# flavie-yuan-liu/DL_attack_on_ImageNet

Measured on AMD Instinct MI355X. Metric: adversarial images/sec (ADiL learning step, classifier included), higher is better.
Workload: dtype bf16; 1 GPU; ADiL learn_dictionary_a step vs resnet50, 512 images/GPU, 50 atoms, 224x224, bf16 image streams + fp32 D/V master, loss=logits, clean pseudo-labels computed once per image and cached (1 fwd + 1 bwd per step; result-neutral, profiles/r03_label_stability.md); global_batch=512, atoms=50, inner_iters=131, parallelism=dp1: images+codes sharded, D replicated, 1 all-reduce(grad_d)/step

## Files before the change

### dl_attack_on_imagenet_amd/_lib.py

```python
import ctypes
import os
from ctypes import c_float, c_int, c_size_t, c_void_p

_PKG = os.path.dirname(os.path.abspath(__file__))
LIBPATH = os.environ.get("ADIL_HIP_LIBRARY") or os.path.join(_PKG, "lib", "libadil_hip.so")

SIGNATURES = {
    "adil_abi_version": (c_int, []),
    "adil_max_atoms": (c_int, []),
    "adil_grad_workspace_bytes": (c_size_t, [c_int, c_int, c_int]),
    "adil_grad_code_rows": (c_int, [c_int]),
    "adil_grad_slab_offset": (c_size_t, [c_int, c_int, c_int]),
    "adil_pack_codes": (c_int, [c_void_p, c_void_p, c_int, c_int, c_void_p, c_void_p, c_void_p, c_int, c_void_p, c_int, c_int,
                                c_void_p]),
    "adil_gather_images": (c_int, [c_void_p, c_int, c_void_p, c_void_p, c_int, c_int, c_int, c_void_p]),
    "adil_spd_inverse": (c_int, [c_void_p, c_int, c_void_p, c_void_p]),
    "adil_synth": (c_int, [c_void_p, c_void_p, c_void_p, c_void_p, c_int, c_int, c_int, c_int, c_float, c_int, c_void_p]),
    "adil_images_to_u8": (c_int, [c_void_p, c_int, c_void_p, c_size_t, c_void_p, c_void_p]),
    "adil_synth_store": (c_int, [c_void_p, c_void_p, c_void_p, c_void_p, c_void_p, c_int, c_int, c_int, c_int, c_float, c_int,
                                 c_void_p]),
    "adil_synth_fp8": (c_int, [c_void_p, c_void_p, c_void_p, c_void_p, c_int, c_int, c_int, c_int, c_float, c_float, c_int,
                               c_void_p]),
    "adil_dict_to_fp8": (c_int, [c_void_p, c_size_t, c_void_p, c_void_p]),
    "adil_adamw_clamp_fp8": (c_int, [c_void_p, c_void_p, c_int, c_void_p, c_void_p, c_size_t, c_float, c_float, c_float,
                                     c_float, c_float, c_float, c_float, c_float, c_void_p, c_void_p, c_void_p, c_void_p]),
    "adil_synth_fp8_packed": (c_int, [c_void_p, c_void_p, c_void_p, c_void_p, c_int, c_int, c_int, c_int, c_float, c_float,
                                      c_int, c_void_p]),
    "adil_grad": (c_int, [c_void_p, c_void_p, c_void_p, c_void_p, c_void_p, c_void_p, c_int, c_int, c_int, c_int, c_int,
                          c_void_p, c_size_t, c_void_p, c_void_p]),
    "adil_adamw_clamp": (c_int, [c_void_p, c_void_p, c_int, c_void_p, c_void_p, c_size_t, c_float, c_float, c_float,
                                 c_float, c_float, c_float, c_float, c_float, c_void_p, c_void_p, c_void_p]),
    "adil_zstep": (c_int, [c_void_p, c_void_p, c_void_p, c_void_p, c_void_p, c_int, c_int, c_int, c_float, c_float,
                           c_float, c_float, c_float, c_float, c_float, c_float, c_void_p, c_void_p, c_float, c_void_p,
                           c_void_p, c_void_p]),
    "adil_zstep_codes_slab_bytes": (c_size_t, [c_int, c_int, c_int]),
    "adil_zstep_codes": (c_int, [c_void_p, c_void_p, c_void_p, c_void_p, c_void_p, c_int, c_int, c_int, c_float, c_float,
                                 c_float, c_float, c_float, c_float, c_float, c_float, c_void_p, c_void_p, c_float, c_void_p,
                                 c_void_p, c_void_p, c_size_t, c_void_p, c_void_p]),
    "adil_adamw_l1ball": (c_int, [c_void_p, c_void_p, c_void_p, c_int, c_void_p, c_void_p, c_int, c_int, c_float, c_float,
                                  c_float, c_float, c_float, c_float, c_float, c_void_p, c_void_p, c_float, c_void_p, c_void_p,
                                  c_void_p, c_int, c_int, c_void_p]),
    "adil_atom_l1ball_project": (c_int, [c_void_p, c_int, c_int, c_int, c_float, c_void_p]),
    "adil_l1ball_project": (c_int, [c_void_p, c_int, c_int, c_float, c_void_p]),
    "adil_l2ball_project": (c_int, [c_void_p, c_int, c_int, c_float, c_void_p]),
    "adil_ista_step": (c_int, [c_void_p, c_void_p, c_size_t, c_float, c_float, c_void_p]),
    "adil_atom_workspace_bytes": (c_size_t, [c_int, c_int]),
    "adil_atom_norms": (c_int, [c_void_p, c_int, c_int, c_void_p, c_void_p, c_size_t, c_void_p]),
    "adil_atom_scale": (c_int, [c_void_p, c_int, c_int, c_void_p, c_int, c_void_p]),
    "adil_gram_workspace_bytes": (c_size_t, [c_int, c_int]),
    "adil_gram": (c_int, [c_void_p, c_int, c_int, c_void_p, c_void_p, c_size_t, c_void_p]),
    "adil_dict_rightmul": (c_int, [c_void_p, c_void_p, c_int, c_int, c_void_p, c_void_p]),
    "adil_image_metrics": (c_int, [c_void_p, c_void_p, c_int, c_int, c_int, c_void_p, c_void_p, c_void_p]),
    "adil_affine_act_fwd": (c_int, [c_void_p, c_void_p, c_void_p, c_void_p, c_void_p, c_size_t, c_int, c_int, c_int, c_int,
                                    c_void_p]),
    "adil_affine_act_bwd": (c_int, [c_void_p, c_void_p, c_void_p, c_void_p, c_void_p, c_size_t, c_int, c_int, c_int, c_int,
                                    c_void_p]),
    "adil_stem_conv_fwd": (c_int, [c_void_p, c_int, c_void_p, c_float, c_float, c_float, c_float, c_float, c_float,
                                   c_void_p, c_void_p, c_void_p, c_int, c_int, c_int, c_void_p]),
    "adil_maxpool_fwd": (c_int, [c_void_p, c_void_p, c_void_p, c_int, c_int, c_int, c_int, c_void_p]),
    "adil_stem_pool_bwd": (c_int, [c_void_p, c_void_p, c_void_p, c_void_p, c_void_p, c_int, c_int, c_int, c_int, c_void_p]),
    "adil_pw_conv_fwd": (c_int, [c_void_p, c_void_p, c_void_p, c_void_p, c_void_p, c_void_p, c_int, c_int, c_int, c_int,
                                 c_void_p, c_void_p, c_int, c_int, c_void_p]),
    "adil_pw_conv_bwd": (c_int, [c_void_p, c_void_p, c_void_p, c_void_p, c_void_p, c_void_p, c_void_p, c_int, c_int, c_int,
                                 c_int, c_void_p, c_void_p, c_void_p, c_void_p, c_int, c_int, c_void_p]),
    "adil_pw_conv_bwd_tile": (c_int, [c_void_p, c_void_p, c_void_p, c_void_p, c_void_p, c_void_p, c_void_p, c_int, c_int, c_int,
                                      c_int, c_void_p, c_void_p, c_void_p, c_void_p, c_int, c_int, c_void_p, c_int]),
    "adil_pw_route_policy": (c_int, [c_int]),
    "adil_pw_join_fwd": (c_int, [c_void_p, c_void_p, c_void_p, c_void_p, c_void_p, c_void_p, c_void_p, c_void_p, c_void_p,
                                 c_void_p, c_void_p, c_void_p, c_int, c_int, c_int, c_void_p]),
    "adil_pw_join_bwd": (c_int, [c_void_p, c_void_p, c_void_p, c_void_p, c_void_p, c_void_p, c_void_p, c_void_p, c_void_p,
                                 c_void_p, c_void_p, c_void_p, c_void_p, c_int, c_int, c_int, c_void_p]),
    "adil_conv3x3": (c_int, [c_void_p, c_void_p, c_void_p, c_int, c_int, c_int, c_int, c_int, c_void_p]),
    "adil_conv3x3_loop": (c_int, [c_int]),
    "adil_conv3x3_s2_fwd": (c_int, [c_void_p, c_void_p, c_void_p, c_int, c_int, c_int, c_int, c_int, c_void_p]),
    "adil_conv3x3_s2_bwd": (c_int, [c_void_p, c_void_p, c_void_p, c_int, c_int, c_int, c_int, c_int, c_void_p]),
    "adil_dw3x3_fwd": (c_int, [c_void_p, c_void_p, c_void_p, c_void_p, c_int, c_int, c_int, c_int, c_int, c_int, c_void_p]),
    "adil_dw3x3_bwd": (c_int, [c_void_p, c_void_p, c_void_p, c_void_p, c_int, c_int, c_int, c_int, c_int, c_int, c_void_p]),
    "adil_pw8_fwd": (c_int, [c_void_p, c_void_p, c_void_p, c_void_p, c_void_p, c_void_p, c_int, c_int, c_int, c_int, c_void_p]),
    "adil_pw8_bwd": (c_int, [c_void_p, c_void_p, c_void_p, c_void_p, c_void_p, c_int, c_int, c_int, c_int, c_void_p]),
    "adil_stem_conv_bwd": (c_int, [c_void_p, c_void_p, c_float, c_float, c_float, c_void_p, c_int, c_int, c_int, c_int,
                                   c_void_p]),
    "adil_first3x3_fwd": (c_int, [c_void_p, c_int, c_void_p, c_float, c_float, c_float, c_float, c_float, c_float,
                                  c_void_p, c_void_p, c_void_p, c_int, c_int, c_int, c_int, c_void_p]),
    "adil_first3x3_bwd": (c_int, [c_void_p, c_void_p, c_void_p, c_void_p, c_float, c_float, c_float, c_void_p, c_int, c_int,
                                  c_int, c_int, c_int, c_void_p]),
    "adil_pool_head_fwd": (c_int, [c_void_p, c_void_p, c_void_p, c_void_p, c_void_p, c_int, c_int, c_int, c_int, c_void_p]),
    "adil_pool_head_bwd": (c_int, [c_void_p, c_void_p, c_void_p, c_void_p, c_int, c_int, c_int, c_int, c_void_p]),
    "adil_bn_pool_head_fwd": (c_int, [c_void_p] * 7 + [c_int, c_int, c_int, c_int, c_void_p]),
    "adil_bn_pool_head_bwd": (c_int, [c_void_p] * 7 + [c_int, c_int, c_int, c_int, c_void_p]),
    "adil_dense1x1_fwd": (c_int, [c_void_p, c_void_p, c_void_p, c_void_p, c_void_p, c_void_p, c_void_p, c_int, c_int, c_int,
                                  c_int, c_void_p]),
    "adil_dense1x1_bwd": (c_int, [c_void_p, c_void_p, c_void_p, c_void_p, c_void_p, c_void_p, c_void_p, c_void_p, c_int, c_int,
                                  c_int, c_int, c_void_p]),
    "adil_dense3x3_fwd": (c_int, [c_void_p, c_void_p, c_void_p, c_int, c_int, c_int, c_int, c_int, c_void_p]),
    "adil_dense3x3_bwd": (c_int, [c_void_p, c_void_p, c_void_p, c_int, c_int, c_int, c_int, c_int, c_void_p]),
    "adil_dense1x1_fwd_ld": (c_int, [c_void_p, c_int, c_void_p, c_void_p, c_void_p, c_void_p, c_void_p, c_void_p, c_int, c_int,
                                     c_int, c_int, c_int, c_void_p]),
    "adil_dense1x1_bwd_ld": (c_int, [c_void_p, c_int, c_void_p, c_int, c_void_p, c_void_p, c_void_p, c_int, c_void_p, c_void_p,
                                     c_void_p, c_int, c_int, c_int, c_int, c_int, c_int, c_void_p]),
    "adil_dense3x3_fwd_ld": (c_int, [c_void_p, c_int, c_void_p, c_void_p, c_int, c_int, c_int, c_int, c_int, c_int, c_void_p]),
    "adil_dense3x3_bwd_ld": (c_int, [c_void_p, c_int, c_void_p, c_void_p, c_int, c_int, c_int, c_int, c_int, c_int, c_void_p]),
    "adil_dense_transition_fwd": (c_int, [c_void_p, c_void_p, c_void_p, c_void_p, c_void_p, c_int, c_int, c_int, c_int, c_int,
                                          c_void_p]),
    "adil_dense_transition_bwd": (c_int, [c_void_p, c_int, c_void_p, c_void_p, c_void_p, c_void_p, c_void_p, c_int, c_int,
                                          c_int, c_int, c_int, c_void_p]),
}

ABI_VERSION = 8
_lib = None


class AdilLibraryError(RuntimeError):
    pass


def load(path: str = None) -> ctypes.CDLL:
    global _lib
    if _lib is not None and path is None:
        return _lib
    p = path or LIBPATH
    import torch
    if not os.path.exists(p):
        raise AdilLibraryError(
            f"HIP kernel library not found at {p}. Build it with `python -m dl_attack_on_imagenet_amd.build` "
            "(needs hipcc). There is no CPU fallback for the ADiL hot path.")
    try:
        lib = ctypes.CDLL(p)
    except OSError as e:
        raise AdilLibraryError(f"cannot load {p}: {e}") from e
    for name, (res, args) in SIGNATURES.items():
        try:
            fn = getattr(lib, name)
        except AttributeError as e:
            raise AdilLibraryError(f"{p} does not export `{name}` (stale build?)") from e
        fn.restype, fn.argtypes = res, args
    if lib.adil_abi_version() != ABI_VERSION:
        raise AdilLibraryError(f"ABI mismatch: library {lib.adil_abi_version()} != binding {ABI_VERSION}")
    if path is None:
        _lib = lib
    return lib


def check(rc: int, what: str) -> None:
    if rc != 0:
        names = {-1: "ADIL_EINVAL (bad argument)", -2: "ADIL_EWORKSPACE (workspace too small)"}
        raise AdilLibraryError(f"{what} failed: {names.get(rc, f'hipError_t {rc}')}")
```

### dl_attack_on_imagenet_amd/csrc/adil_stem.hip

```cpp
#include <hip/hip_runtime.h>
#include <stdint.h>

#include "adil_common.h"
#include "adil_hip.h"
#include "adil_mfma.h"

namespace {

struct StemNorm { float mean[3]; float inv_std[3]; };

#define ST_T 16
#define ST_ROWS (2 * ST_T + 5)
#define ST_COLS 40
#define ST_RS (ST_COLS * 4 + 8)
#define ST_K 224
#define ST_WS (ST_K + 8)
#define ST_OS 72

template <typename TX>
__global__ __launch_bounds__(256) __attribute__((amdgpu_waves_per_eu(3))) void stem_conv_fwd_kernel(const TX* __restrict__ x, const bf16_t* __restrict__ wf,
                                                            StemNorm nm, const float* __restrict__ scale,
                                                            const float* __restrict__ shift, bf16_t* __restrict__ y,
                                                            int H, int W, int OH, int OW) {
    __shared__ __attribute__((aligned(16))) bf16_t smem[ST_ROWS * ST_RS + 64 * ST_WS];
    static_assert(4 * 32 * ST_OS <= ST_ROWS * ST_RS + 64 * ST_WS, "output scratch must fit in the tile buffers");
    bf16_t* sin = smem;
    bf16_t* sw = smem + ST_ROWS * ST_RS;
    bf16_t* sout = smem;
    const int tid = threadIdx.x, lane = tid & 63, w = tid >> 6, c = lane & 31, h = lane >> 5;
    const int n = blockIdx.z, oh0 = blockIdx.y * ST_T, ow0 = blockIdx.x * ST_T;
    {
        u32x4 wv[7];
#pragma unroll
        for (int j = 0; j < 7; ++j) wv[j] = *reinterpret_cast<const u32x4*>(wf + (size_t)(tid + 256 * j) * 8);
#pragma unroll
        for (int j = 0; j < 7; ++j) {
            const int q = tid + 256 * j, co = q / 28, off = q - co * 28;
            *reinterpret_cast<u32x4*>(sw + co * ST_WS + off * 8) = wv[j];
        }
    }
    const TX* xn = x + (size_t)n * 3 * H * W;
    constexpr int NPOS = (ST_ROWS * ST_COLS + 255) / 256;
    float raw[NPOS][3], okm[NPOS];
#pragma unroll
    for (int j = 0; j < NPOS; ++j) {
        const int pos = tid + 256 * j < ST_ROWS * ST_COLS ? tid + 256 * j : ST_ROWS * ST_COLS - 1;
        const int row = pos / ST_COLS, col = pos - row * ST_COLS;
        const int ih = 2 * oh0 - 3 + row, iw = 2 * ow0 - 3 + col;
        const bool ok = (ih >= 0) && (ih < H) && (iw >= 0) && (iw < W);
        const size_t at = (size_t)(ok ? ih : 0) * W + (ok ? iw : 0);
        okm[j] = ok ? 1.0f : 0.0f;
        raw[j][0] = Elem<TX>::load(xn, at);
        raw[j][1] = Elem<TX>::load(xn + (size_t)H * W, at);
        raw[j][2] = Elem<TX>::load(xn + (size_t)2 * H * W, at);
    }
#pragma unroll
    for (int j = 0; j < NPOS; ++j) {
        const int pos = tid + 256 * j;
        const int row = pos / ST_COLS, col = pos - row * ST_COLS;
        const float v0 = (raw[j][0] - nm.mean[0]) * nm.inv_std[0] * okm[j];
        const float v1 = (raw[j][1] - nm.mean[1]) * nm.inv_std[1] * okm[j];
        const float v2 = (raw[j][2] - nm.mean[2]) * nm.inv_std[2] * okm[j];
        u32x2 t;
        t[0] = pack2_bf16(v0, v1);
        t[1] = pack2_bf16(v2, 0.0f);
        if (pos < ST_ROWS * ST_COLS) *reinterpret_cast<u32x2*>(sin + row * ST_RS + col * 4) = t;
    }
    lds_sync();
    f32x16 acc[2][2];
#pragma unroll
    for (int p = 0; p < 2; ++p)
#pragma unroll
        for (int ct = 0; ct < 2; ++ct)
#pragma unroll
            for (int r = 0; r < 16; ++r) acc[p][ct][r] = 0.0f;
    const int prow = c >> 4, pcol = c & 15;
#pragma unroll 1
    for (int kh = 0; kh < 7; ++kh) {
#pragma unroll
        for (int g = 0; g < 2; ++g) {
            bf16x8 a[2], b[2];
#pragma unroll
            for (int ct = 0; ct < 2; ++ct) a[ct] = lds8(sw + (ct * 32 + c) * ST_WS + kh * 32 + 16 * g + 8 * h);
#pragma unroll
            for (int p = 0; p < 2; ++p) {
                const int orow = 2 * (2 * w + p) + prow;
                b[p] = lds8(sin + (2 * orow + kh) * ST_RS + 8 * pcol + 16 * g + 8 * h);
            }
#pragma unroll
            for (int p = 0; p < 2; ++p)
#pragma unroll
                for (int ct = 0; ct < 2; ++ct) mma16(acc[p][ct], a[ct], b[p]);
        }
    }
    lds_sync();
    bf16_t* so = sout + w * 32 * ST_OS;
#pragma unroll
    for (int p = 0; p < 2; ++p) {
#pragma unroll
        for (int ct = 0; ct < 2; ++ct) {
#pragma unroll
            for (int q = 0; q < 4; ++q) {
                const int co = ct * 32 + 8 * q + 4 * h;
                float v[4];
#pragma unroll
                for (int j = 0; j < 4; ++j) v[j] = fmaxf(acc[p][ct][4 * q + j] * scale[co + j] + shift[co + j], 0.0f);
                u32x2 t;
                t[0] = pack2_bf16(v[0], v[1]);
                t[1] = pack2_bf16(v[2], v[3]);
                *reinterpret_cast<u32x2*>(so + c * ST_OS + co) = t;
            }
        }
#pragma unroll
        for (int i = 0; i < 4; ++i) {
            const int id = lane + 64 * i, px = id >> 3, ch = (id & 7) * 8;
            const int oh = oh0 + 2 * (2 * w + p) + (px >> 4), ow = ow0 + (px & 15);
            const u32x4 t = *reinterpret_cast<const u32x4*>(so + px * ST_OS + ch);
            if (oh < OH && ow < OW) *reinterpret_cast<u32x4*>(y + (((size_t)n * OH + oh) * OW + ow) * 64 + ch) = t;
        }
    }
}


__global__ __launch_bounds__(256) void maxpool_fwd_kernel(const bf16_t* __restrict__ y, bf16_t* __restrict__ p,
                                                          uint8_t* __restrict__ idx, int B, int OH, int OW, int PH, int PW,
                                                          int C8) {
    const size_t i = (size_t)blockIdx.x * 256 + threadIdx.x;
    const size_t total = (size_t)B * PH * PW * C8;
    if (i >= total) return;
    const int c8 = (int)(i % C8);
    size_t r = i / C8;
    const int pw = (int)(r % PW); r /= PW;
    const int ph = (int)(r % PH);
    const int n = (int)(r / PH);
    float best[8];
    unsigned bi[8];
#pragma unroll
    for (int j = 0; j < 8; ++j) { best[j] = -INFINITY; bi[j] = 0xffu; }
#pragma unroll
    for (int kh = 0; kh < 3; ++kh) {
        const int oh = 2 * ph - 1 + kh;
#pragma unroll
        for (int kw = 0; kw < 3; ++kw) {
            const int ow = 2 * pw - 1 + kw;
            if (oh >= 0 && oh < OH && ow >= 0 && ow < OW) {
                const u32x4 t = *reinterpret_cast<const u32x4*>(y + ((((size_t)n * OH + oh) * OW + ow) * C8 + c8) * 8);
                float f[8];
                unpack8(t, f);
#pragma unroll
                for (int j = 0; j < 8; ++j) {
                    const bool take = (f[j] > best[j]) || (f[j] != f[j]) || (bi[j] == 0xffu);
                    best[j] = take ? f[j] : best[j];
                    bi[j] = take ? (unsigned)(kh * 3 + kw) : bi[j];
                }
            }
        }
    }
    *reinterpret_cast<u32x4*>(p + i * 8) = pack8(best);
    u32x2 o;
    o[0] = bi[0] | (bi[1] << 8) | (bi[2] << 16) | (bi[3] << 24);
    o[1] = bi[4] | (bi[5] << 8) | (bi[6] << 16) | (bi[7] << 24);
    *reinterpret_cast<u32x2*>(idx + i * 8) = o;
}

__global__ __launch_bounds__(256) void stem_pool_bwd_kernel(const bf16_t* __restrict__ g, const uint8_t* __restrict__ idx,
                                                            const bf16_t* __restrict__ p, const float* __restrict__ scale,
                                                            bf16_t* __restrict__ gy, int B, int OH, int OW, int PH, int PW,
                                                            int C8) {
    const size_t i = (size_t)blockIdx.x * 256 + threadIdx.x;
    const size_t total = (size_t)B * OH * OW * C8;
    if (i >= total) return;
    const int c8 = (int)(i % C8);
    size_t r = i / C8;
    const int ow = (int)(r % OW); r /= OW;
    const int oh = (int)(r % OH);
    const int n = (int)(r / OH);
    float acc[8];
#pragma unroll
    for (int j = 0; j < 8; ++j) acc[j] = 0.0f;
    const int ph0 = oh >> 1, nph = 1 + (oh & 1), pw0 = ow >> 1, npw = 1 + (ow & 1);
    for (int a = 0; a < nph; ++a) {
        const int ph = ph0 + a;
        if (ph >= PH) continue;
        const int kh = oh - (2 * ph - 1);
        for (int b = 0; b < npw; ++b) {
            const int pw = pw0 + b;
            if (pw >= PW) continue;
            const unsigned want = (unsigned)(kh * 3 + (ow - (2 * pw - 1)));
            const size_t at = ((((size_t)n * PH + ph) * PW + pw) * C8 + c8) * 8;
            const u32x2 id = *reinterpret_cast<const u32x2*>(idx + at);
            const u32x4 gt = *reinterpret_cast<const u32x4*>(g + at);
            const u32x4 pt = *reinterpret_cast<const u32x4*>(p + at);
            float gf[8], pf[8];
            unpack8(gt, gf);
            unpack8(pt, pf);
#pragma unroll
            for (int j = 0; j < 8; ++j) {
                const unsigned k = (id[j >> 2] >> (8 * (j & 3))) & 0xffu;
                acc[j] += (k == want && pf[j] > 0.0f) ? gf[j] : 0.0f;
            }
        }
    }
#pragma unroll
    for (int j = 0; j < 8; ++j) acc[j] *= scale[c8 * 8 + j];
    *reinterpret_cast<u32x4*>(gy + i * 8) = pack8(acc);
}

#define SB_TH 16
#define SB_TW 32
#define SB_GR (SB_TH / 2 + 3)
#define SB_GC (SB_TW / 2 + 3)
#define SB_PS 72

typedef float f32x4 __attribute__((ext_vector_type(4)));

template <int A, int BB>
__device__ __forceinline__ void stem_bwd_class(f32x4 (&acc)[2], const bf16_t* sg, const bf16_t* swb, int w, int l16, int ks) {
    const int wrow = (l16 < 3 ? l16 : 0) * 49 * 64;
    const bool wlane = l16 < 3;
#pragma unroll 1
    for (int kh = 1 - A; kh < 7; kh += 2) {
#pragma unroll
        for (int kw = 1 - BB; kw < 7; kw += 2) {
            const int col = l16 + (BB + 3 - kw) / 2 + 1;
#pragma unroll
            for (int cg = 0; cg < 2; ++cg) {
                bf16x8 a = {};
                if (wlane) a = lds8(swb + wrow + (kh * 7 + kw) * 64 + 32 * cg + 8 * ks);
#pragma unroll
                for (int q = 0; q < 2; ++q) {
                    const int row = 2 * w + q + (A + 3 - kh) / 2 + 1;
                    const bf16x8 b = lds8(sg + (row * SB_GC + col) * SB_PS + 32 * cg + 8 * ks);
                    acc[q] = __builtin_amdgcn_mfma_f32_16x16x32_bf16(a, b, acc[q], 0, 0, 0);
                }
            }
        }
    }
}

template <typename TX> __device__ __forceinline__ void st_pair(TX* p, float a, float b);
template <> __device__ __forceinline__ void st_pair<float>(float* p, float a, float b) {
    *reinterpret_cast<float2*>(p) = make_float2(a, b);
}
template <> __device__ __forceinline__ void st_pair<bf16_t>(bf16_t* p, float a, float b) {
    *reinterpret_cast<unsigned*>(p) = pack2_bf16(a, b);
}

template <typename TX>
__global__ __launch_bounds__(256) __attribute__((amdgpu_waves_per_eu(3))) void stem_conv_bwd_kernel(const bf16_t* __restrict__ gy, const bf16_t* __restrict__ wb,
                                                            StemNorm nm, TX* __restrict__ gx, int H, int W, int OH,
                                                            int OW) {
    __shared__ __attribute__((aligned(16))) bf16_t sg[SB_GR * SB_GC * SB_PS];
    __shared__ __attribute__((aligned(16))) bf16_t swb[3 * 49 * 64];
    const int tid = threadIdx.x, lane = tid & 63, w = tid >> 6, c = lane & 31, h = lane >> 5;
    const int n = blockIdx.z, ih0 = blockIdx.y * SB_TH, iw0 = blockIdx.x * SB_TW;
    {
        constexpr int NWQ = (3 * 49 * 8 + 255) / 256, NGQ = (SB_GR * SB_GC * 8 + 255) / 256;
        u32x4 wv[NWQ], gv[NGQ];
        bool gok[NGQ];
#pragma unroll
        for (int j = 0; j < NWQ; ++j) {
            const int q = tid + 256 * j < 3 * 49 * 8 ? tid + 256 * j : 3 * 49 * 8 - 1;
            wv[j] = *reinterpret_cast<const u32x4*>(wb + q * 8);
        }
        const int ohb = ih0 / 2 - 1, owb = iw0 / 2 - 1;
#pragma unroll
        for (int j = 0; j < NGQ; ++j) {
            const int q = tid + 256 * j < SB_GR * SB_GC * 8 ? tid + 256 * j : SB_GR * SB_GC * 8 - 1;
            const int ch = q & 7, px = q >> 3;
            const int row = px / SB_GC, col = px - row * SB_GC;
            const int oh = ohb + row, ow = owb + col;
            gok[j] = (oh >= 0) && (oh < OH) && (ow >= 0) && (ow < OW);
            gv[j] = *reinterpret_cast<const u32x4*>(gy + (((size_t)n * OH + (gok[j] ? oh : 0)) * OW + (gok[j] ? ow : 0)) * 64 + ch * 8);
        }
#pragma unroll
        for (int j = 0; j < NWQ; ++j) {
            const int q = tid + 256 * j;
            if (q < 3 * 49 * 8) *reinterpret_cast<u32x4*>(swb + q * 8) = wv[j];
        }
#pragma unroll
        for (int j = 0; j < NGQ; ++j) {
            const int q = tid + 256 * j;
            const int ch = q & 7, px = q >> 3;
            u32x4 t = gv[j];
            if (!gok[j]) t = u32x4{0u, 0u, 0u, 0u};
            if (q < SB_GR * SB_GC * 8) *reinterpret_cast<u32x4*>(sg + px * SB_PS + ch * 8) = t;
        }
    }
    lds_sync();
    const int l16 = lane & 15, ks = lane >> 4;
    f32x4 acc[4][2];
#pragma unroll
    for (int k = 0; k < 4; ++k)
#pragma unroll
        for (int q = 0; q < 2; ++q) acc[k][q] = f32x4{0.0f, 0.0f, 0.0f, 0.0f};
    stem_bwd_class<0, 0>(acc[0], sg, swb, w, l16, ks);
    stem_bwd_class<0, 1>(acc[1], sg, swb, w, l16, ks);
    stem_bwd_class<1, 0>(acc[2], sg, swb, w, l16, ks);
    stem_bwd_class<1, 1>(acc[3], sg, swb, w, l16, ks);
    if (ks == 0) {
        const int iw = iw0 + 2 * l16;
#pragma unroll
        for (int q = 0; q < 2; ++q) {
#pragma unroll
            for (int a = 0; a < 2; ++a) {
                const int ih = ih0 + 2 * (2 * w + q) + a;
                if (ih < H && iw < W) {
#pragma unroll
                    for (int ci = 0; ci < 3; ++ci) {
                        TX* o = gx + (((size_t)n * 3 + ci) * H + ih) * W + iw;
                        st_pair<TX>(o, acc[2 * a][q][ci] * nm.inv_std[ci], acc[2 * a + 1][q][ci] * nm.inv_std[ci]);
                    }
                }
            }
        }
    }
}

}

extern "C" int adil_stem_conv_fwd(const void* x, int x_dtype, const void* w_fwd, float mean0, float mean1, float mean2,
                                  float inv_std0, float inv_std1, float inv_std2, const float* scale, const float* shift,
                                  void* y, int B, int H, int W, void* stream) {
    ADIL_ENTER();
    if (!x || !w_fwd || !scale || !shift || !y || B <= 0 || B > 65535 || H <= 0 || W <= 0 || (H & 1) || (W & 1)) return ADIL_EINVAL;
    if (x_dtype != ADIL_F32 && x_dtype != ADIL_BF16) return ADIL_EINVAL;
    const StemNorm nm = {{mean0, mean1, mean2}, {inv_std0, inv_std1, inv_std2}};
    const int OH = H / 2, OW = W / 2;
    const dim3 grid((OW + ST_T - 1) / ST_T, (OH + ST_T - 1) / ST_T, B);
    hipStream_t st = (hipStream_t)stream;
    if (x_dtype == ADIL_F32)
        hipLaunchKernelGGL(stem_conv_fwd_kernel<float>, grid, dim3(256), 0, st, (const float*)x, (const bf16_t*)w_fwd, nm,
                           scale, shift, (bf16_t*)y, H, W, OH, OW);
    else
        hipLaunchKernelGGL(stem_conv_fwd_kernel<bf16_t>, grid, dim3(256), 0, st, (const bf16_t*)x, (const bf16_t*)w_fwd, nm,
                           scale, shift, (bf16_t*)y, H, W, OH, OW);
    ADIL_CHECK_LAUNCH();
    return 0;
}

extern "C" int adil_maxpool_fwd(const void* y, void* p, uint8_t* idx, int B, int OH, int OW, int C, void* stream) {
    ADIL_ENTER();
    if (!y || !p || !idx || B <= 0 || OH <= 0 || OW <= 0 || C <= 0 || (C & 7)) return ADIL_EINVAL;
    const int PH = (OH - 1) / 2 + 1, PW = (OW - 1) / 2 + 1;
    const size_t total = (size_t)B * PH * PW * (C / 8);
    hipLaunchKernelGGL(maxpool_fwd_kernel, dim3((unsigned)((total + 255) / 256)), dim3(256), 0, (hipStream_t)stream,
                       (const bf16_t*)y, (bf16_t*)p, idx, B, OH, OW, PH, PW, C / 8);
    ADIL_CHECK_LAUNCH();
    return 0;
}

extern "C" int adil_stem_pool_bwd(const void* g, const uint8_t* idx, const void* p, const float* scale, void* gy, int B,
                                  int OH, int OW, int C, void* stream) {
    ADIL_ENTER();
    if (!g || !idx || !p || !scale || !gy || B <= 0 || OH <= 0 || OW <= 0 || C <= 0 || (C & 7)) return ADIL_EINVAL;
    const int PH = (OH - 1) / 2 + 1, PW = (OW - 1) / 2 + 1;
    const size_t total = (size_t)B * OH * OW * (C / 8);
    hipLaunchKernelGGL(stem_pool_bwd_kernel, dim3((unsigned)((total + 255) / 256)), dim3(256), 0, (hipStream_t)stream,
                       (const bf16_t*)g, idx, (const bf16_t*)p, scale, (bf16_t*)gy, B, OH, OW, PH, PW, C / 8);
    ADIL_CHECK_LAUNCH();
    return 0;
}

extern "C" int adil_stem_conv_bwd(const void* gy, const void* w_bwd, float inv_std0, float inv_std1, float inv_std2, void* gx,
                                  int gx_dtype, int B, int H, int W, void* stream) {
    ADIL_ENTER();
    if (!gy || !w_bwd || !gx || B <= 0 || B > 65535 || H <= 0 || W <= 0 || (H & 1) || (W & 1)) return ADIL_EINVAL;
    if (gx_dtype != ADIL_F32 && gx_dtype != ADIL_BF16) return ADIL_EINVAL;
    const StemNorm nm = {{0.0f, 0.0f, 0.0f}, {inv_std0, inv_std1, inv_std2}};
    const int OH = H / 2, OW = W / 2;
    const dim3 grid((W + SB_TW - 1) / SB_TW, (H + SB_TH - 1) / SB_TH, B);
    hipStream_t st = (hipStream_t)stream;
    if (gx_dtype == ADIL_F32)
        hipLaunchKernelGGL(stem_conv_bwd_kernel<float>, grid, dim3(256), 0, st, (const bf16_t*)gy, (const bf16_t*)w_bwd, nm,
                           (float*)gx, H, W, OH, OW);
    else
        hipLaunchKernelGGL(stem_conv_bwd_kernel<bf16_t>, grid, dim3(256), 0, st, (const bf16_t*)gy, (const bf16_t*)w_bwd, nm,
                           (bf16_t*)gx, H, W, OH, OW);
    ADIL_CHECK_LAUNCH();
    return 0;
}
```

### include/adil_hip.h

```cpp
#ifndef ADIL_HIP_H
#define ADIL_HIP_H

#include <stddef.h>
#include <stdint.h>

#ifdef __cplusplus
extern "C" {
#endif

#define ADIL_F32 0
#define ADIL_BF16 1
#define ADIL_U8 2

#define ADIL_EINVAL (-1)
#define ADIL_EWORKSPACE (-2)

int adil_abi_version(void);

int adil_max_atoms(void);

size_t adil_grad_workspace_bytes(int B, int P, int K);

int adil_grad_code_rows(int K);

size_t adil_grad_slab_offset(int B, int P, int K);

int adil_pack_codes(const float* v, const int64_t* index, int B, int K, float* vp, int32_t* pos, void* vpt,
                    int vpt_dtype, const float* slabs, int nslabs, int slab_rows, void* stream);

int adil_gather_images(const void* src, int src_dtype, const int64_t* index, void* dst, int dst_dtype, int B, int P,
                       void* stream);

int adil_images_to_u8(const void* src, int src_dtype, uint8_t* dst, size_t n, unsigned long long* mismatches, void* stream);

int adil_synth(const void* x, const float* d, const float* vp, void* out, int B, int P, int K, int dtype,
               float delta_clamp, int pixel_clamp, void* stream);

int adil_synth_store(const uint8_t* store, const int64_t* index, const float* d, const float* vp, void* out, int B, int P,
                     int K, int out_dtype, float delta_clamp, int pixel_clamp, void* stream);

int adil_synth_fp8(const void* x, const float* d, const float* vp, void* out, int B, int P, int K, int dtype,
                   float v_absmax, float delta_clamp, int pixel_clamp, void* stream);

int adil_dict_to_fp8(const float* d, size_t n, void* d_fp8, void* stream);
int adil_adamw_clamp_fp8(float* p, const void* g, int g_dtype, float* m, float* s, size_t n, float decay, float b1,
                         float b2, float eps, float step_size, float bc2_sqrt, float lo, float hi, float* max_abs_delta,
                         const float* dyn_scalars, void* p_fp8, void* stream);
int adil_synth_fp8_packed(const void* x, const void* d_fp8, const float* vp, void* out, int B, int P, int K, int dtype,
                          float v_absmax, float delta_clamp, int pixel_clamp, void* stream);

int adil_grad(const void* g, const float* d, const float* vp, const void* vpt, float* grad_d, float* grad_vb, int B, int P,
              int K, int dtype, int accumulate_d, void* ws, size_t ws_bytes, int* nslabs_out, void* stream);

int adil_adamw_clamp(float* p, const void* g, int g_dtype, float* m, float* s, size_t n, float decay, float b1,
                     float b2, float eps, float step_size, float bc2_sqrt, float lo, float hi,
                     float* max_abs_delta, const float* dyn_scalars, void* stream);

int adil_zstep(float* z, float* m, float* s, const float* dpinv_t, const float* gvp, int B, int P, int K, float decay,
               float b1, float b2, float eps, float step_size, float bc2_sqrt, float lo, float hi, float* max_abs_delta,
               const float* skip_if_below, float skip_threshold, float* clear, const float* dyn_scalars, void* stream);

size_t adil_zstep_codes_slab_bytes(int B, int P, int K);
int adil_zstep_codes(float* z, float* m, float* s, const float* dpinv_t, const float* gvp, int B, int P, int K, float decay,
                     float b1, float b2, float eps, float step_size, float bc2_sqrt, float lo, float hi, float* max_abs_delta,
                     const float* skip_if_below, float skip_threshold, float* clear, const float* dyn_scalars,
                     float* code_slabs, size_t code_slab_bytes, int* nslabs_out, void* stream);

int adil_adamw_l1ball(float* v, const float* grad_vb, int32_t* pos, int reset_pos, float* m, float* s, int N, int K,
                      float decay, float b1, float b2, float eps, float step_size, float bc2_sqrt, float radius,
                      float* max_abs_delta, const float* skip_if_below, float skip_threshold, float* clear,
                      const float* dyn_scalars, const float* slabs, int nslabs, int slab_rows, void* stream);

int adil_atom_l1ball_project(float* d, int C, int HW, int K, float radius, void* stream);

int adil_l1ball_project(float* x, int N, int K, float radius, void* stream);

int adil_l2ball_project(float* x, int N, int K, float radius, void* stream);

int adil_ista_step(float* v, const float* g, size_t n, float step, float lam, void* stream);

size_t adil_atom_workspace_bytes(int P, int K);
int adil_atom_norms(const float* d, int P, int K, float* norms, void* ws, size_t ws_bytes, void* stream);

int adil_atom_scale(float* d, int P, int K, const float* norms, int sphere, void* stream);

size_t adil_gram_workspace_bytes(int P, int K);
int adil_gram(const float* d, int P, int K, float* gram, void* ws, size_t ws_bytes, void* stream);

int adil_spd_inverse(const float* a, int K, float* out, void* stream);

int adil_dict_rightmul(const float* d, const float* mat, int P, int K, float* out, void* stream);

int adil_image_metrics(const void* adv, const void* x, int B, int P, int dtype, float* sq_err, float* sq_norm,
                       void* stream);

int adil_affine_act_fwd(const void* x, const void* res, const float* scale, const float* shift, void* y, size_t n, int C,
                        int inner, int relu, int dtype, void* stream);
int adil_affine_act_bwd(const void* g, const void* y, const float* scale, void* gx, void* gres, size_t n, int C,
                        int inner, int relu, int dtype, void* stream);

int adil_stem_conv_fwd(const void* x, int x_dtype, const void* w_fwd, float mean0, float mean1, float mean2, float inv_std0,
                       float inv_std1, float inv_std2, const float* scale, const float* shift, void* y, int B, int H, int W,
                       void* stream);
int adil_maxpool_fwd(const void* y, void* p, uint8_t* idx, int B, int OH, int OW, int C, void* stream);
int adil_stem_pool_bwd(const void* g, const uint8_t* idx, const void* p, const float* scale, void* gy, int B, int OH, int OW,
                       int C, void* stream);
int adil_stem_conv_bwd(const void* gy, const void* w_bwd, float inv_std0, float inv_std1, float inv_std2, void* gx,
                       int gx_dtype, int B, int H, int W, void* stream);

int adil_pw_conv_fwd(const void* x, const void* w, const float* scale, const float* shift, const void* res, void* y, int M,
                     int K, int N, int relu, const float* pscale, const float* pshift, int sub_w, int sub_hw, void* stream);
int adil_pw_conv_bwd(const void* g, const void* g2, const void* y, const float* scale, const void* wt, void* gx, void* gres,
                     int M, int K, int N, int relu, const void* xin, const float* pscale, const float* pshift, const void* g3,
                     int sub_w, int sub_hw, void* stream);
int adil_pw_conv_bwd_tile(const void* g, const void* g2, const void* y, const float* scale, const void* wt, void* gx,
                          void* gres, int M, int K, int N, int relu, const void* xin, const float* pscale,
                          const float* pshift, const void* g3, int sub_w, int sub_hw, void* stream, int bo);
int adil_pw_route_policy(int policy);
int adil_conv3x3_loop(int variant);

int adil_pw_join_fwd(const void* h2raw, const float* pscale2, const float* pshift2, const void* w3, const float* scale3,
                     const float* shift3, const void* res, void* out, const void* w1, const float* scale1,
                     const float* shift1, void* h1, int M, int W, int C, void* stream);
int adil_pw_join_bwd(const void* g_h1, const void* h1, const float* scale1, const void* wt1, const void* g_out,
                     const void* out, const float* scale3, void* gres, const void* wt3, const void* h2raw,
                     const float* pscale2, const float* pshift2, void* gx, int M, int W, int C, void* stream);

int adil_conv3x3(const void* x, const void* wp, void* y, int B, int H, int W, int C, int N, void* stream);

#define ADIL_CONV3X3_S2_MAX_W 63
int adil_conv3x3_s2_fwd(const void* x, const void* wp, void* y, int B, int H, int W, int C, int N, void* stream);
int adil_conv3x3_s2_bwd(const void* g, const void* wp_bwd, void* gx, int B, int H, int W, int C, int N, void* stream);

int adil_dw3x3_fwd(const void* x, const float* w, const float* bias, void* y, int B, int H, int W, int C, int stride,
                   int relu6, void* stream);
int adil_dw3x3_bwd(const void* g, const void* y, const float* w, void* gx, int B, int H, int W, int C, int stride,
                   int relu6, void* stream);

int adil_pw8_fwd(const void* x, const void* w, const float* scale, const float* shift, const void* res, void* y, int M,
                 int K, int N, int act, void* stream);
int adil_pw8_bwd(const void* g, const void* y, const float* scale, const void* wt, void* gx, int M, int K, int N, int act,
                 void* stream);

int adil_first3x3_fwd(const void* x, int x_dtype, const void* w_fwd, float mean0, float mean1, float mean2, float inv_std0,
                      float inv_std1, float inv_std2, const float* scale, const float* shift, void* y, int B, int H, int W,
                      int relu6, void* stream);
int adil_first3x3_bwd(const void* g, const void* y, const float* scale, const void* w_bwd, float inv_std0, float inv_std1,
                      float inv_std2, void* gx, int gx_dtype, int B, int H, int W, int relu6, void* stream);

int adil_pool_head_fwd(const void* x, const float* wt, const float* bias, float* pooled, float* logits, int B, int HW,
                       int C, int N, void* stream);
int adil_pool_head_bwd(const float* g, const float* w, float* gpooled, void* gx, int B, int HW, int C, int N, void* stream);

int adil_bn_pool_head_fwd(const void* x, const float* pscale, const float* pshift, const float* wt, const float* bias,
                          float* pooled, float* logits, int B, int HW, int C, int N, void* stream);
int adil_bn_pool_head_bwd(const float* g, const float* w, const void* x, const float* pscale, const float* pshift,
                          float* gpooled, void* gx, int B, int HW, int C, int N, void* stream);

int adil_dense1x1_fwd(const void* x, const float* pscale, const float* pshift, const void* w, const float* scale,
                      const float* shift, void* y, int M, int K, int N, int act, void* stream);
int adil_dense1x1_bwd(const void* g, const void* y, const float* scale, const void* wt, const void* xin, const float* pscale,
                      const float* pshift, void* gx, int M, int K, int N, int act, void* stream);
int adil_dense1x1_fwd_ld(const void* x, int ldx, const float* pscale, const float* pshift, const void* w,
                         const float* scale, const float* shift, void* y, int ldy,
                         int M, int K, int N, int act, void* stream);
int adil_dense1x1_bwd_ld(const void* g, int ldg, const void* y, int ldy, const float* scale, const void* wt,
                         const void* xin, int ldxin, const float* pscale, const float* pshift,
                         void* gx, int ldgx, int accumulate, int M, int K, int N, int act, void* stream);

#define ADIL_DENSE3X3_MAX_W 63
int adil_dense3x3_fwd(const void* x, const void* wp, void* y, int B, int H, int W, int C, int N, void* stream);
int adil_dense3x3_bwd(const void* g, const void* wp_bwd, void* gx, int B, int H, int W, int C, int N, void* stream);
int adil_dense3x3_fwd_ld(const void* x, int ldx, const void* wp, void* y, int ldy,
                         int B, int H, int W, int C, int N, void* stream);
int adil_dense3x3_bwd_ld(const void* g, int ldg, const void* wp_bwd, void* gx, int ldgx,
                         int B, int H, int W, int C, int N, void* stream);

int adil_dense_transition_fwd(const void* x, const float* pscale, const float* pshift, const void* w, void* y,
                              int B, int H, int W, int K, int N, void* stream);
int adil_dense_transition_bwd(const void* g, int ldg, const void* wt, const void* xin, const float* pscale,
                              const float* pshift, void* gx, int B, int H, int W, int K, int N, void* stream);

#ifdef __cplusplus
}
#endif
#endif
```

Measured before the change: 24550 images/sec.

## Add quad-gather stem pool backward and persistent shifted-tap stem conv backward

Adds a maxpool-backward kernel in which each thread owns a 2x2 quad of pooled outputs and gathers the contributions to four pre-pool pixels, replacing the per-output scatter/gather. It also adds a persistent stem conv-backward kernel that loops over tiles, prefetches the next gradient tile into registers while MFMAs run on the current one, and restructures the 7x7 stride-2 transpose as shifted taps with a software-pipelined LDS fragment load. Both kernels are the default through a new variant switch, and the old kernels remain as fallbacks. This adds complexity and risks correctness at tile and pooling edges.

```diff
diff --git a/dl_attack_on_imagenet_amd/_lib.py b/dl_attack_on_imagenet_amd/_lib.py
--- a/dl_attack_on_imagenet_amd/_lib.py
+++ b/dl_attack_on_imagenet_amd/_lib.py
@@ -80,6 +80,7 @@
     "adil_pw8_bwd": (c_int, [c_void_p, c_void_p, c_void_p, c_void_p, c_void_p, c_int, c_int, c_int, c_int, c_void_p]),
     "adil_stem_conv_bwd": (c_int, [c_void_p, c_void_p, c_float, c_float, c_float, c_void_p, c_int, c_int, c_int, c_int,
                                    c_void_p]),
+    "adil_stem_bwd_variant": (c_int, [c_int]),
     "adil_first3x3_fwd": (c_int, [c_void_p, c_int, c_void_p, c_float, c_float, c_float, c_float, c_float, c_float,
                                   c_void_p, c_void_p, c_void_p, c_int, c_int, c_int, c_int, c_void_p]),
     "adil_first3x3_bwd": (c_int, [c_void_p, c_void_p, c_void_p, c_void_p, c_float, c_float, c_float, c_void_p, c_int, c_int,
diff --git a/dl_attack_on_imagenet_amd/csrc/adil_stem.hip b/dl_attack_on_imagenet_amd/csrc/adil_stem.hip
--- a/dl_attack_on_imagenet_amd/csrc/adil_stem.hip
+++ b/dl_attack_on_imagenet_amd/csrc/adil_stem.hip
@@ -317,6 +317,195 @@
     }
 }
 
+__global__ __launch_bounds__(256) void stem_pool_bwd_quad_kernel(const bf16_t* __restrict__ g, const uint8_t* __restrict__ idx,
+                                                                 const bf16_t* __restrict__ p, const float* __restrict__ scale,
+                                                                 bf16_t* __restrict__ gy, int OH, int OW, int PH, int PW,
+                                                                 int C8) {
+    const unsigned j = blockIdx.y * 256u + threadIdx.x;
+    if (j >= (unsigned)PW * (unsigned)C8) return;
+    const int b = (int)(j / (unsigned)C8), c8 = (int)(j - (unsigned)b * (unsigned)C8);
+    const int n = (int)(blockIdx.x / (unsigned)PH), a = (int)(blockIdx.x - (unsigned)n * (unsigned)PH);
+    const bool oka = a + 1 < PH, okb = b + 1 < PW;
+    const int a1 = oka ? a + 1 : a, b1 = okb ? b + 1 : b;
+    const size_t r0 = ((size_t)n * PH + a) * PW, r1 = ((size_t)n * PH + a1) * PW;
+    const size_t at[4] = {((r0 + b) * C8 + c8) * 8, ((r0 + b1) * C8 + c8) * 8, ((r1 + b) * C8 + c8) * 8,
+                          ((r1 + b1) * C8 + c8) * 8};
+    u32x2 id[4];
+    u32x4 gt[4], pt[4];
+#pragma unroll
+    for (int k = 0; k < 4; ++k) {
+        id[k] = *reinterpret_cast<const u32x2*>(idx + at[k]);
+        gt[k] = *reinterpret_cast<const u32x4*>(g + at[k]);
+        pt[k] = *reinterpret_cast<const u32x4*>(p + at[k]);
+    }
+    const bool okw[4] = {true, okb, oka, oka && okb};
+    float sc[8];
+#pragma unroll
+    for (int jj = 0; jj < 8; ++jj) sc[jj] = scale[c8 * 8 + jj];
+    float gf[4][8];
+    bool pos[4][8];
+    unsigned kk[4][8];
+#pragma unroll
+    for (int k = 0; k < 4; ++k) {
+        float pf[8];
+        unpack8(gt[k], gf[k]);
+        unpack8(pt[k], pf);
+#pragma unroll
+        for (int jj = 0; jj < 8; ++jj) {
+            kk[k][jj] = (id[k][jj >> 2] >> (8 * (jj & 3))) & 0xffu;
+            pos[k][jj] = okw[k] && pf[jj] > 0.0f;
+        }
+    }
+#pragma unroll
+    for (int dy = 0; dy < 2; ++dy) {
+#pragma unroll
+        for (int dx = 0; dx < 2; ++dx) {
+            const int oh = 2 * a + dy, ow = 2 * b + dx;
+            float acc[8];
+#pragma unroll
+            for (int jj = 0; jj < 8; ++jj) acc[jj] = 0.0f;
+#pragma unroll
+            for (int wy = 0; wy <= dy; ++wy) {
+#pragma unroll
+                for (int wx = 0; wx <= dx; ++wx) {
+                    const int k = 2 * wy + wx;
+                    const unsigned want = (unsigned)((dy + 1 - 2 * wy) * 3 + (dx + 1 - 2 * wx));
+#pragma unroll
+                    for (int jj = 0; jj < 8; ++jj) acc[jj] += (kk[k][jj] == want && pos[k][jj]) ? gf[k][jj] : 0.0f;
+                }
+            }
+#pragma unroll
+            for (int jj = 0; jj < 8; ++jj) acc[jj] *= sc[jj];
+            if (oh < OH && ow < OW)
+                *reinterpret_cast<u32x4*>(gy + ((((size_t)n * OH + oh) * OW + ow) * C8 + c8) * 8) = pack8(acc);
+        }
+    }
+}
+
+#define SQ_PS 80
+#define SQ_WKH (7 * 64 + 8)
+#define SQ_WCI (7 * SQ_WKH + 24)
+#define SQ_WN (2 * SQ_WCI + 6 * SQ_WKH + 7 * 64)
+
+template <typename TX>
+__global__ __launch_bounds__(256) __attribute__((amdgpu_waves_per_eu(3))) void stem_conv_bwd_shift_kernel(
+    const bf16_t* __restrict__ gy, const bf16_t* __restrict__ wb, StemNorm nm, TX* __restrict__ gx, int H, int W, int OH,
+    int OW, int NTX, int NTY, int ntiles) {
+    __shared__ __attribute__((aligned(16))) bf16_t sg[SB_GR * SB_GC * SQ_PS];
+    __shared__ __attribute__((aligned(16))) bf16_t swb[SQ_WN + 8];
+    const int tid = threadIdx.x, lane = tid & 63, w = tid >> 6;
+    constexpr int NWQ = (3 * 49 * 8 + 255) / 256, NGQ = (SB_GR * SB_GC * 8 + 255) / 256;
+    const int t0 = (int)((long long)blockIdx.x * ntiles / gridDim.x), t1 = (int)((long long)(blockIdx.x + 1) * ntiles / gridDim.x);
+    int n, ih0, iw0;
+    u32x4 gv[NGQ];
+    unsigned gok = 0;
+    auto tile_load = [&](int t, int& tn, int& tih0, int& tiw0) {
+        const int tx = t % NTX, r = t / NTX;
+        tn = r / NTY;
+        tih0 = (r - tn * NTY) * SB_TH;
+        tiw0 = tx * SB_TW;
+        const int ohb = tih0 / 2 - 1, owb = tiw0 / 2 - 1;
+        gok = 0;
+#pragma unroll
+        for (int j = 0; j < NGQ; ++j) {
+            const int q = tid + 256 * j < SB_GR * SB_GC * 8 ? tid + 256 * j : SB_GR * SB_GC * 8 - 1;
+            const int ch = q & 7, px = q >> 3;
+            const int row = px / SB_GC, col = px - row * SB_GC;
+            const int oh = ohb + row, ow = owb + col;
+            const bool ok = (oh >= 0) && (oh < OH) && (ow >= 0) && (ow < OW);
+            gok |= ok ? 1u << j : 0u;
+            gv[j] = *reinterpret_cast<const u32x4*>(gy + (((size_t)tn * OH + (ok ? oh : 0)) * OW + (ok ? ow : 0)) * 64 + ch * 8);
+        }
+    };
+    auto tile_to_lds = [&]() {
+#pragma unroll
+        for (int j = 0; j < NGQ; ++j) {
+            const int q = tid + 256 * j;
+            const int ch = q & 7, px = q >> 3;
+            u32x4 t = gv[j];
+            if (!(gok >> j & 1u)) t = u32x4{0u, 0u, 0u, 0u};
+            if (q < SB_GR * SB_GC * 8) *reinterpret_cast<u32x4*>(sg + px * SQ_PS + ch * 8) = t;
+        }
+    };
+    {
+        u32x4 wv[NWQ];
+#pragma unroll
+        for (int j = 0; j < NWQ; ++j) {
+            const int q = tid + 256 * j < 3 * 49 * 8 ? tid + 256 * j : 3 * 49 * 8 - 1;
+            wv[j] = *reinterpret_cast<const u32x4*>(wb + q * 8);
+        }
+        tile_load(t0, n, ih0, iw0);
+#pragma unroll
+        for (int j = 0; j < NWQ; ++j) {
+            const int q = tid + 256 * j;
+            const int ci = q / (49 * 8), r = q - ci * 49 * 8, tap = r >> 3, ch = r & 7, kh = tap / 7, kw = tap - kh * 7;
+            if (q < 3 * 49 * 8) *reinterpret_cast<u32x4*>(swb + ci * SQ_WCI + kh * SQ_WKH + kw * 64 + ch * 8) = wv[j];
+        }
+        if (tid == 0) *reinterpret_cast<u32x4*>(swb + SQ_WN) = u32x4{0u, 0u, 0u, 0u};
+        tile_to_lds();
+    }
+    lds_sync();
+    const int l16 = lane & 15, ks = lane >> 4;
+    const int ci = l16 & 3, ca = l16 >> 3, cb = (l16 >> 2) & 1;
+    const int abase = (ci < 3 ? ci : 0) * SQ_WCI + (ca + 3) * SQ_WKH + (cb + 3) * 64 + 8 * ks;
+    const bool okc = ci < 3, oka = okc && ca == 1, okb = okc && cb == 1, okab = oka && cb == 1;
+    const int bbase = ((2 * w + 1) * SB_GC + l16 + 1) * SQ_PS + 8 * ks;
+#pragma unroll 1
+    for (int t = t0; t < t1; ++t) {
+        int nn = 0, nih0 = 0, niw0 = 0;
+        if (t + 1 < t1) tile_load(t + 1, nn, nih0, niw0);
+        f32x4 acc[2];
+        acc[0] = f32x4{0.0f, 0.0f, 0.0f, 0.0f};
+        acc[1] = f32x4{0.0f, 0.0f, 0.0f, 0.0f};
+        constexpr int SQ_AHEAD = 2;
+        bf16x8 fa[SQ_AHEAD + 1], fb[SQ_AHEAD + 1][2];
+#pragma unroll
+        for (int s = 0; s < 32 + SQ_AHEAD; ++s) {
+            if (s < 32) {
+                const int dr = 2 - (s >> 3), dc = 2 - ((s >> 1) & 3), cg = s & 1, f = s % (SQ_AHEAD + 1);
+                const bool ok = dr == 2 ? (dc == 2 ? okab : oka) : (dc == 2 ? okb : okc);
+                fa[f] = lds8(swb + (ok ? abase - 2 * dr * SQ_WKH - 2 * dc * 64 + 32 * cg : SQ_WN));
+#pragma unroll
+                for (int q = 0; q < 2; ++q) fb[f][q] = lds8(sg + bbase + ((q + dr) * SB_GC + dc) * SQ_PS + 32 * cg);
+            }
+            if (s >= SQ_AHEAD) {
+                const int f = (s - SQ_AHEAD) % (SQ_AHEAD + 1);
+#pragma unroll
+                for (int q = 0; q < 2; ++q) acc[q] = __builtin_amdgcn_mfma_f32_16x16x32_bf16(fa[f], fb[f][q], acc[q], 0, 0, 0);
+            }
+        }
+        const int iw = iw0 + 2 * l16;
+#pragma unroll
+        for (int q = 0; q < 2; ++q) {
+            const int ih = ih0 + 2 * (2 * w + q) + (ks >> 1);
+            float v[3], o[3];
+#pragma unroll
+            for (int c = 0; c < 3; ++c) {
+                v[c] = acc[q][c] * nm.inv_std[c];
+                o[c] = __shfl_down(v[c], 16);
+            }
+            if (!(ks & 1) && ih < H && iw < W) {
+#pragma unroll
+                for (int c = 0; c < 3; ++c) st_pair<TX>(gx + (((size_t)n * 3 + c) * H + ih) * W + iw, v[c], o[c]);
+            }
+        }
+        if (t + 1 < t1) {
+            lds_sync();
+            tile_to_lds();
+            n = nn; ih0 = nih0; iw0 = niw0;
+            lds_sync();
+        }
+    }
+}
+
+static int g_stem_bwd_variant = 0;
+
+}
+
+extern "C" int adil_stem_bwd_variant(int variant) {
+    const int prev = g_stem_bwd_variant;
+    if (variant == 0 || variant == 1) g_stem_bwd_variant = variant;
+    return prev;
 }
 
 extern "C" int adil_stem_conv_fwd(const void* x, int x_dtype, const void* w_fwd, float mean0, float mean1, float mean2,
@@ -355,6 +544,13 @@
     ADIL_ENTER();
     if (!g || !idx || !p || !scale || !gy || B <= 0 || OH <= 0 || OW <= 0 || C <= 0 || (C & 7)) return ADIL_EINVAL;
     const int PH = (OH - 1) / 2 + 1, PW = (OW - 1) / 2 + 1;
+    const long long rows = (long long)B * PH, cols = ((long long)PW * (C / 8) + 255) / 256;
+    if (g_stem_bwd_variant == 0 && rows <= 0x7fffffffLL && cols <= 65535) {
+        hipLaunchKernelGGL(stem_pool_bwd_quad_kernel, dim3((unsigned)rows, (unsigned)cols), dim3(256), 0, (hipStream_t)stream,
+                           (const bf16_t*)g, idx, (const bf16_t*)p, scale, (bf16_t*)gy, OH, OW, PH, PW, C / 8);
+        ADIL_CHECK_LAUNCH();
+        return 0;
+    }
     const size_t total = (size_t)B * OH * OW * (C / 8);
     hipLaunchKernelGGL(stem_pool_bwd_kernel, dim3((unsigned)((total + 255) / 256)), dim3(256), 0, (hipStream_t)stream,
                        (const bf16_t*)g, idx, (const bf16_t*)p, scale, (bf16_t*)gy, B, OH, OW, PH, PW, C / 8);
@@ -371,6 +567,19 @@
     const int OH = H / 2, OW = W / 2;
     const dim3 grid((W + SB_TW - 1) / SB_TW, (H + SB_TH - 1) / SB_TH, B);
     hipStream_t st = (hipStream_t)stream;
+    const long long ntiles = (long long)grid.x * grid.y * B;
+    if (g_stem_bwd_variant == 0 && ntiles <= 0x7fffffffLL) {
+        const long long slots = 3LL * adil_num_cu();
+        const dim3 lin((unsigned)(ntiles < slots ? ntiles : slots));
+        if (gx_dtype == ADIL_F32)
+            hipLaunchKernelGGL(stem_conv_bwd_shift_kernel<float>, lin, dim3(256), 0, st, (const bf16_t*)gy, (const bf16_t*)w_bwd, nm,
+                               (float*)gx, H, W, OH, OW, (int)grid.x, (int)grid.y, (int)ntiles);
+        else
+            hipLaunchKernelGGL(stem_conv_bwd_shift_kernel<bf16_t>, lin, dim3(256), 0, st, (const bf16_t*)gy, (const bf16_t*)w_bwd,
+                               nm, (bf16_t*)gx, H, W, OH, OW, (int)grid.x, (int)grid.y, (int)ntiles);
+        ADIL_CHECK_LAUNCH();
+        return 0;
+    }
     if (gx_dtype == ADIL_F32)
         hipLaunchKernelGGL(stem_conv_bwd_kernel<float>, grid, dim3(256), 0, st, (const bf16_t*)gy, (const bf16_t*)w_bwd, nm,
                            (float*)gx, H, W, OH, OW);
diff --git a/include/adil_hip.h b/include/adil_hip.h
--- a/include/adil_hip.h
+++ b/include/adil_hip.h
@@ -107,6 +107,7 @@
                        int C, void* stream);
 int adil_stem_conv_bwd(const void* gy, const void* w_bwd, float inv_std0, float inv_std1, float inv_std2, void* gx,
                        int gx_dtype, int B, int H, int W, void* stream);
+int adil_stem_bwd_variant(int variant);
 
 int adil_pw_conv_fwd(const void* x, const void* w, const float* scale, const float* shift, const void* res, void* y, int M,
                      int K, int N, int relu, const float* pscale, const float* pshift, int sub_w, int sub_hw, void* stream);
```

Result: faster. 25710 images/sec (median of 6 runs) (+4.7%).
